# ustcml/RecStudio

Measured on AMD Instinct MI355X. Metric: M scored (user,pos,neg) triplets/sec at d=128, higher is better.
Workload: dtype f32; 1 GPU; BPR two-tower d=128, synthetic 10000001 items / 1000001 users / 1e8-interaction Zipf popularity, positives uniform over the items it holds, popular sampler neg=64, InnerProduct + BPR loss, B=65536 queries/step (BASELINE.json configs[1]); global_batch=65536, num_neg=64, dim=128, n_items=10000001, parallelism=single

## Files before the change

include/recstudio_amd.h:

```cpp
#ifndef RECSTUDIO_AMD_H
#define RECSTUDIO_AMD_H

#include <stdint.h>

#ifdef __cplusplus
extern "C" {
#endif

#define RSA_ABI_VERSION 12

typedef void* rsa_stream_t;

enum rsa_status {
  RSA_OK = 0,
  RSA_ERR_ARG = -1,
  RSA_ERR_HIP = -2,
  RSA_ERR_UNSUPPORTED = -3
};

enum rsa_score_mode { RSA_SCORE_IP = 0, RSA_SCORE_COS = 1, RSA_SCORE_EUC = 2  };
enum rsa_sampler_kind { RSA_SAMPLER_GIVEN = 0, RSA_SAMPLER_UNIFORM = 1, RSA_SAMPLER_POPULAR = 2 };
enum rsa_loss_kind { RSA_LOSS_BPR = 0, RSA_LOSS_SSM = 1, RSA_LOSS_BCE = 2,
                      RSA_LOSS_WBPR = 3, RSA_LOSS_WBCE = 4, RSA_LOSS_HINGE = 5, RSA_LOSS_NCE = 6,
                     RSA_LOSS_CCL = 7 };
// ... 197 lines not shown
  int32_t _pad;
  const rsa_popular_args* pop;
  uint64_t seed, offset;
  uint32_t grid_threads;
  uint32_t _pad2;
  uint64_t elem_base;
  const float* step_scale;
  int64_t* neg_ids;
  uint8_t* solo;
  void* item_workspace;
  int64_t item_workspace_bytes;
  void* user_workspace;
  int64_t user_workspace_bytes;
  float* pos_score;
  float* neg_score;
  float* row_loss;
  float* dpos;
  float* dneg;
  float* query_grad;
  const float* ones;
  float* loss_out;
  void* reduce_scratch;
  int64_t uniform_high;
} rsa_bpr_sgd_args;
int rsa_bpr_sgd_prepare(const rsa_bpr_sgd_args* args, rsa_stream_t stream);
int rsa_bpr_sgd_apply(const rsa_bpr_sgd_args* args, rsa_stream_t stream);

int rsa_scatter_add_rows(const float* src, const int64_t* ids, int64_t numel, int32_t dim,
                         float* dst, int64_t n_rows, rsa_stream_t stream);

typedef struct rsa_seg_gather_args {
  int64_t size;
  const float* item_table;
  int64_t n_items;
  int32_t dim;
  int32_t max_len;
  const int64_t* flat_item_ids;
  int64_t n_flat;
  const int64_t* seg_start;
  const int64_t* seg_end;
  int64_t n_seg;
  int64_t* out_ids;
  float* out_rows;
  int64_t* out_len;
} rsa_seg_gather_args;
int rsa_seg_gather(const rsa_seg_gather_args* args, rsa_stream_t stream);

int rsa_row_sqnorm(const float* table, int64_t n_rows, int32_t dim, int32_t score_mode, float* out, rsa_stream_t stream);

// ... 212 lines not shown
```

recstudio_amd/_native.py:

```python
import ctypes
import os
import subprocess
from ctypes import (POINTER, Structure, c_char_p, c_double, c_float, c_int, c_int32, c_int64, c_uint32, c_uint64, c_void_p)

HERE = os.path.dirname(os.path.abspath(__file__))
LIB_PATH = os.environ.get('RSA_LIB') or os.path.join(HERE, 'librecstudio_amd.so')
CSRC = os.path.join(HERE, 'csrc')

RSA_OK = 0
SCORE_IP, SCORE_COS, SCORE_EUC = 0, 1, 2
SAMPLER_GIVEN, SAMPLER_UNIFORM, SAMPLER_POPULAR = 0, 1, 2
LOSS_BPR, LOSS_SSM, LOSS_BCE = 0, 1, 2
LOSS_WBPR, LOSS_WBCE, LOSS_HINGE, LOSS_NCE, LOSS_CCL = 3, 4, 5, 6, 7


class NativeError(RuntimeError):
    """A C-ABI call returned a negative status."""


class FusedArgs(Structure):
    _fields_ = [
        ('item_table', c_void_p), ('n_items', c_int64), ('dim', c_int32), ('score_mode', c_int32),
        ('query', c_void_p), ('query_index', c_void_p), ('n_query_rows', c_int64),
        ('pos_ids', c_void_p), ('n_queries', c_int64),
# ... 92 lines not shown
    ]


class RowsUpdateArgs(_Sized):
    _fields_ = [
        ('size', c_int64), ('query', c_void_p), ('query_index', c_void_p), ('n_query_rows', c_int64), ('dim', c_int32),
        ('has_pos', c_int32), ('pos_ids', c_void_p), ('neg_ids', c_void_p), ('n_queries', c_int64), ('num_neg', c_int32),
        ('_pad', c_int32), ('dpos', c_void_p), ('dneg', c_void_p), ('upstream', c_void_p), ('n_items', c_int64),
        ('pad_row', c_int64), ('target', c_void_p), ('exp_avg', c_void_p), ('exp_avg_sq', c_void_p), ('lr', c_double),
        ('beta1', c_double), ('beta2', c_double), ('eps', c_double), ('step', c_int64), ('solo', c_void_p), ('workspace', c_void_p),
        ('workspace_bytes', c_int64),
    ]


class BprSgdArgs(_Sized):
    _fields_ = [
        ('size', c_int64), ('item_table', c_void_p), ('n_items', c_int64), ('user_table', c_void_p), ('n_users', c_int64),
        ('dim', c_int32), ('num_neg', c_int32), ('user_ids', c_void_p), ('pos_ids', c_void_p), ('n_queries', c_int64),
        ('sampler', c_int32), ('_pad', c_int32), ('pop', POINTER(PopularArgs)), ('seed', c_uint64), ('offset', c_uint64),
        ('grid_threads', c_uint32), ('_pad2', c_uint32), ('elem_base', c_uint64), ('step_scale', c_void_p), ('neg_ids', c_void_p),
        ('solo', c_void_p), ('item_workspace', c_void_p), ('item_workspace_bytes', c_int64), ('user_workspace', c_void_p),
        ('user_workspace_bytes', c_int64), ('pos_score', c_void_p), ('neg_score', c_void_p), ('row_loss', c_void_p),
        ('dpos', c_void_p), ('dneg', c_void_p), ('query_grad', c_void_p), ('ones', c_void_p), ('loss_out', c_void_p),
        ('reduce_scratch', c_void_p), ('uniform_high', c_int64),
    ]


class SegGatherArgs(_Sized):
    _fields_ = [
        ('size', c_int64), ('item_table', c_void_p), ('n_items', c_int64), ('dim', c_int32), ('max_len', c_int32),
        ('flat_item_ids', c_void_p), ('n_flat', c_int64), ('seg_start', c_void_p), ('seg_end', c_void_p), ('n_seg', c_int64),
        ('out_ids', c_void_p), ('out_rows', c_void_p), ('out_len', c_void_p),
    ]


class FullscoreArgs(_Sized):
    _fields_ = [
        ('size', c_int64), ('item_table', c_void_p), ('n_items', c_int64), ('dim', c_int32), ('score_mode', c_int32),
        ('query', c_void_p), ('n_query', c_int64), ('scores', c_void_p), ('lse', c_void_p), ('topk_val', c_void_p),
        ('topk_idx', c_void_p), ('k', c_int32), ('_pad', c_int32), ('item_aux', c_void_p), ('query_aux', c_void_p),
        ('workspace', c_void_p), ('workspace_bytes', c_int64),
    ]


STRUCTS = {
    'rsa_fused_args': FusedArgs, 'rsa_backward_args': BackwardArgs, 'rsa_shard_route_args': ShardRouteArgs,
    'rsa_shard_home_args': ShardHomeArgs, 'rsa_shard_backward_args': ShardBackwardArgs,
# ... 13 lines not shown
    'rsa_sample_popular': (c_int, [POINTER(PopularArgs), c_void_p]),
    'rsa_popular_lookup': (c_int, [POINTER(PopularArgs), c_void_p]),
    'rsa_item_logp': (c_int, [c_void_p, c_int64, c_void_p, c_int64, c_void_p, c_void_p]),
    'rsa_embedding_gather': (c_int, [c_void_p, c_int64, c_int32, c_void_p, c_int64, c_void_p, c_void_p]),
    'rsa_fused_sample_gather_score': (c_int, [POINTER(FusedArgs), c_void_p]),
    'rsa_pairwise_loss': (c_int, [POINTER(LossArgs), c_void_p]),
    'rsa_ssm_shared_loss': (c_int, [POINTER(LossArgs), c_void_p]),
    'rsa_mean_rows': (c_int, [c_void_p, c_int64, c_void_p, c_void_p, c_void_p]),
    'rsa_row_lse': (c_int, [c_void_p, c_int64, c_int64, c_void_p, c_void_p, c_float, c_void_p]),
    'rsa_fused_backward': (c_int, [POINTER(BackwardArgs), c_void_p]),
    'rsa_sort_step_elements': (c_int, [POINTER(RowsUpdateArgs), c_void_p]),
    'rsa_rows_update_presorted': (c_int, [POINTER(RowsUpdateArgs), c_void_p]),
    'rsa_scatter_add_rows': (c_int, [c_void_p, c_void_p, c_int64, c_int32, c_void_p, c_int64, c_void_p]),
    'rsa_seg_gather': (c_int, [POINTER(SegGatherArgs), c_void_p]),
    'rsa_fullscore_softmax': (c_int, [c_void_p, c_int64, c_int32, c_void_p, c_int64, c_void_p, c_void_p, c_void_p,
                                      c_void_p]),
    'rsa_fullscore_softmax_dq_workspace_bytes': (c_int64, [c_int64, c_int64, c_int32]),
    'rsa_fullscore_softmax_dq': (c_int, [c_void_p, c_int64, c_int32, c_void_p, c_int64, c_void_p, c_void_p, c_void_p,
                                         c_void_p, c_void_p, c_int64, c_void_p]),
    'rsa_scatter_rows_sorted_workspace_bytes': (c_int64, [c_int64, c_int32, c_int64]),
    'rsa_rows_update_sorted': (c_int, [POINTER(RowsUpdateArgs), c_void_p]),
    'rsa_bpr_sgd_prepare': (c_int, [POINTER(BprSgdArgs), c_void_p]),
    'rsa_bpr_sgd_apply': (c_int, [POINTER(BprSgdArgs), c_void_p]),
    'rsa_probs_t_query': (c_int, [c_void_p, c_int64, c_int64, c_int64, c_void_p, c_int32, c_void_p, c_void_p]),
    'rsa_fullscore_lse_grad_workspace_bytes': (c_int64, [c_int64, c_int64, c_int32]),
    'rsa_fullscore_lse_grad': (c_int, [c_void_p, c_int64, c_int32, c_void_p, c_int64, c_void_p, c_void_p, c_void_p, c_int64, c_void_p]),
    'rsa_fullscore_softmax_dw': (c_int, [c_void_p, c_int64, c_int32, c_void_p, c_int64, c_void_p, c_void_p, c_void_p, c_void_p]),
    'rsa_rng_advance': (c_int, [c_void_p, c_uint64, c_void_p]),
    'rsa_placement_probe': (c_int, [c_void_p, c_int64, c_void_p, c_int64, c_uint32, c_void_p]),
    'rsa_row_topk': (c_int, [c_void_p, c_int64, c_int64, c_int32, c_void_p, c_void_p, c_void_p]),
    'rsa_topk_mask_history': (c_int, [c_void_p, c_void_p, c_int32, c_void_p, c_int32, c_int64, c_int32, c_void_p,
                                      c_void_p, c_void_p]),
    'rsa_shard_count': (c_int, [c_void_p, c_void_p, c_int64, c_int32, c_int64, c_int32, c_void_p, c_void_p]),
    'rsa_shard_route': (c_int, [c_void_p, c_void_p, c_int64, c_int32, c_int64, c_int32, c_int64, c_void_p, c_void_p,
                                c_void_p, c_void_p]),
    'rsa_shard_segment_stride': (c_int64, [c_int64]),
    'rsa_shard_sample_route': (c_int, [POINTER(ShardRouteArgs), c_void_p]),
    'rsa_shard_route_workgroups': (c_int64, [POINTER(ShardRouteArgs)]),
    'rsa_shard_route_query_groups': (c_int32, [c_int32, c_uint32, c_uint64, c_int32, c_int32]),
    'rsa_shard_score_segments': (c_int, [c_void_p, c_int64, c_int32, c_void_p, c_int64, c_void_p, c_int64, c_int64, c_void_p,
                                         c_void_p, c_void_p, c_void_p]),
    'rsa_shard_home': (c_int, [POINTER(ShardHomeArgs), c_void_p]),
    'rsa_shard_scatter_slots': (c_int, [c_void_p, c_void_p, c_void_p, c_int64, c_int32, c_void_p, c_void_p]),
    'rsa_shard_unpack_segments': (c_int, [c_void_p, c_int64, c_int64, c_void_p, c_void_p, c_void_p, c_void_p, c_void_p,
                                          c_void_p]),
    'rsa_shard_backward_workspace_bytes': (c_int64, [c_int64, c_int64, c_int64]),
# ... 66 lines not shown
```

recstudio_amd/csrc/rsa_internal.hpp:

```cpp
#pragma once
#include "rsa_launch.hpp"

namespace rsa {

struct AdamArgs {
  float* exp_avg;
  float* exp_avg_sq;
  float one_minus_beta1, one_minus_beta2, eps, step_size;
};

struct SortedLayout {
  uint64_t *pairs_a, *pairs_b;
  void* temp;
  float *lead_part, *trail_part;
  int32_t* meta;
};

int64_t sorted_workspace_bytes(int64_t max_total);
SortedLayout sorted_layout(void* workspace, int64_t max_total);

int classify_solo(uint64_t* pairs, int64_t total, int64_t pad_row, int64_t drop_key, uint8_t* solo, hipStream_t s, const char* who);

int apply_sorted_segments(const uint64_t* pairs, int64_t total, int64_t slots, const float* query, int32_t dim,
                          const int64_t* keys, const float* d, const float* upstream, int64_t n_rows, int64_t pad_row,
                          float* target, const SortedLayout& L, hipStream_t s);

struct StepDraw;
int64_t step_all_workspace_bytes(int64_t n_queries, int32_t num_neg);
int sort_step_all(const int64_t* pos_ids, int64_t* neg_ids, const int64_t* user_ids, int64_t n_queries, int32_t num_neg,
                  int64_t n_items, int64_t n_users, uint8_t* solo, void* workspace, int64_t workspace_bytes, const StepDraw* draw,
                  hipStream_t s, const char* who);
int apply_step_all(bool users, const float* query, const int64_t* query_index, int32_t dim, int64_t n_queries, int32_t num_neg,
                   const float* dpos, const float* dneg, const float* upstream, int64_t n_items, int64_t n_users, float* target,
                   void* workspace, hipStream_t s);

int sample_popular(const rsa_popular_args& a, rsa_stream_t stream);

}
```

recstudio_amd/csrc/rsa_sorted.hip:

```cpp
#include "rsa_common.hpp"
#include "rsa_radix.hpp"
#include "rsa_internal.hpp"
#include <cstring>

#ifndef RSA_SORTED_UNROLL
#define RSA_SORTED_UNROLL 4
#endif
#ifndef RSA_SORTED_NT
#define RSA_SORTED_NT 2
#endif

namespace rsa {

template <bool NT>
__device__ __forceinline__ float ld_row(const float* p) {
  if constexpr (NT) return __builtin_nontemporal_load(p);
  return *p;
}
template <bool NT>
__device__ __forceinline__ void st_row(float* p, float v) {
  if constexpr (NT) __builtin_nontemporal_store(v, p);
  else *p = v;
}

template <int NDW, bool NT = false>
__device__ __forceinline__ void apply_run(float* __restrict__ target, const AdamArgs& adam, int32_t cur, float scale, int lane,
                                          const float (&acc)[NDW], const float (&trow)[NDW], const float (&mrow_v)[NDW],
                                          const float (&vrow_v)[NDW]) {
  constexpr int D = 64 * NDW;
  float* row = target + (size_t)cur * D;
  if (adam.exp_avg == nullptr) {
#pragma unroll
// ... 94 lines not shown
  uint64_t work = __ballot(in && !solo && key != drop_key && key != pad_row);
  int last_t = -1;
  constexpr int U = RSA_SORTED_UNROLL;
  while (work) {
    int ts[U];
    int nu = 0;
#pragma unroll
    for (int u = 0; u < U; ++u) {
      ts[u] = 63;
      if (work) {
        ts[u] = __ffsll((unsigned long long)work) - 1;
        work &= work - 1;
        nu = u + 1;
      }
    }
    float qv[U][NDW], tv[U][NDW], mv[U][NDW], vv[U][NDW];
#pragma unroll
    for (int u = 0; u < U; ++u) {
      const int32_t qr = u < nu ? __builtin_amdgcn_readlane(qrow, ts[u]) : 0;
      const int32_t kr = u < nu ? __builtin_amdgcn_readlane(key, ts[u]) : 0;
      const float* qp = query + (size_t)qr * D;
      const float* tp = target + (size_t)kr * D;
#pragma unroll
      for (int k = 0; k < NDW; ++k) {
        qv[u][k] = qp[k * 64 + lane];
        tv[u][k] = ld_row<NT>(tp + k * 64 + lane);
      }
      if (adam.exp_avg != nullptr) {
        const float* mp = adam.exp_avg + (size_t)kr * D;
        const float* vp = adam.exp_avg_sq + (size_t)kr * D;
#pragma unroll
        for (int k = 0; k < NDW; ++k) {
          mv[u][k] = ld_row<NT>(mp + k * 64 + lane);
          vv[u][k] = ld_row<NT>(vp + k * 64 + lane);
        }
      } else {
#pragma unroll
        for (int k = 0; k < NDW; ++k) mv[u][k] = vv[u][k] = 0.f;
      }
    }
#pragma unroll
    for (int u = 0; u < U; ++u) {
      if (u >= nu) break;
      const int t = ts[u];
      const int32_t kt = __builtin_amdgcn_readlane(key, t);
      const int32_t before = t == 0 ? prev : __builtin_amdgcn_readlane(key, t - 1);
      const bool head = kt != before;
      if (head) {
        close_segment();
        cur = kt;
// ... 39 lines not shown
                                                            const int32_t* __restrict__ meta) {
  constexpr int D = 64 * NDW;
  const int lane = lane_id();
  const int64_t chunk = (int64_t)blockIdx.x * 4 + (threadIdx.x >> 6);
  if (chunk >= n_chunks) return;
  const int32_t cur = meta[chunk * META_STRIDE + META_TRAIL_KEY];
  if (cur < 0 || cur == pad_row) return;
  const float scale = upstream ? upstream[0] : 1.f;
  float acc[NDW], trow[NDW], mrow_v[NDW], vrow_v[NDW];
#pragma unroll
  for (int k = 0; k < NDW; ++k) {
    acc[k] = trail_part[(size_t)chunk * D + k * 64 + lane];
    trow[k] = target[(size_t)cur * D + k * 64 + lane];
    mrow_v[k] = adam.exp_avg ? adam.exp_avg[(size_t)cur * D + k * 64 + lane] : 0.f;
    vrow_v[k] = adam.exp_avg ? adam.exp_avg_sq[(size_t)cur * D + k * 64 + lane] : 0.f;
  }
  for (int64_t c2 = chunk + 1; c2 < n_chunks; ++c2) {
    if (meta[c2 * META_STRIDE + META_LEAD_KEY] != cur) break;
#pragma unroll
    for (int k = 0; k < NDW; ++k) acc[k] += lead_part[(size_t)c2 * D + k * 64 + lane];
    if (!meta[c2 * META_STRIDE + META_LEAD_FULL]) break;
  }
  apply_run<NDW>(target, adam, cur, scale, lane, acc, trow, mrow_v, vrow_v);
}

constexpr int32_t SOLO_BIT = (int32_t)0x80000000;
template <bool MOSTLY_SOLO>
__global__ __launch_bounds__(256) void classify_solo_kernel(uint64_t* __restrict__ pairs, int64_t total, int32_t pad_row,
                                                            int32_t drop_key, uint8_t* __restrict__ solo) {
  const int64_t stride = (int64_t)gridDim.x * blockDim.x;
  for (int64_t i = (int64_t)blockIdx.x * blockDim.x + threadIdx.x; i < total; i += stride) {
    const uint64_t pr = pairs[i];
    const int32_t k = (int32_t)rdx_key(pr);
    const int32_t before = i > 0 ? (int32_t)rdx_key(pairs[i - 1]) : -1, after = i + 1 < total ? (int32_t)rdx_key(pairs[i + 1]) : -1;
    const uint32_t e = rdx_val(pr);
    if (k != before && k != after && k != pad_row && k != drop_key) {
      if (!MOSTLY_SOLO) solo[e] = 1;
      pairs[i] = pr | (uint64_t)(uint32_t)SOLO_BIT;
    } else if (MOSTLY_SOLO) {
      solo[e] = 0;
    }
  }
}

constexpr int64_t SORTED_SMALL_TOTAL = 1 << 18;
int sorted_chunk_elems(int64_t total) { return total <= SORTED_SMALL_TOTAL ? 16 : 64; }
// ... 88 lines not shown
                "rsa_scatter_rows_sorted_workspace_bytes(n_queries, num_neg + 1, n_items): the user rows are sorted with the item rows)",
                who, (long long)workspace_bytes, (long long)need);
  const SortedLayout L = sorted_layout(workspace, total);
  const unsigned bits = step_all_bits(n_items, n_users);
  const SrcStepIds it{pos_ids, neg_ids, n_items, num_neg, num_neg + 1, 1};
  const StepDraw none{nullptr, 0, 0, PhiloxCall{0, 0, 1, 0}, 0, 0, nullptr, nullptr, nullptr};
  const SrcStepAll<false> rd{it, user_ids, t_items, n_users, (uint32_t)(n_items + 1), none};
  hipError_t err;
  if (draw != nullptr && draw->kind != 0) {
    const SrcStepAll<true> dw{it, user_ids, t_items, n_users, (uint32_t)(n_items + 1), *draw};
    err = radix_sort_pairs2(dw, rd, L.pairs_a, L.pairs_b, total, bits, L.temp, s);
  } else {
    err = radix_sort_pairs(rd, L.pairs_a, L.pairs_b, total, bits, L.temp, s);
  }
  if (err != hipSuccess) {
    rsa::set_error("%s: radix sort failed: %s", who, hipGetErrorString(hipGetLastError()));
    return RSA_ERR_HIP;
  }
  return classify_solo(radix_result(L.pairs_a, L.pairs_b, bits), t_items, 0, n_items, solo, s, who);
}

int apply_step_all(bool users, const float* query, const int64_t* query_index, int32_t dim, int64_t n_queries, int32_t num_neg,
                   const float* dpos, const float* dneg, const float* upstream, int64_t n_items, int64_t n_users, float* target,
                   void* workspace, hipStream_t s) {
  const int64_t t_items = n_queries * (int64_t)(num_neg + 1), total = t_items + n_queries;
  const SortedLayout L = sorted_layout(workspace, total);
  const uint64_t* sorted = radix_result(L.pairs_a, L.pairs_b, step_all_bits(n_items, n_users));
  const AdamArgs none{nullptr, nullptr, 0.f, 0.f, 0.f, 0.f};
  if (!users) {
    const DecStep dec{query_index, dpos, dneg, (int)num_neg, 1};
    return apply_sorted_pairs(sorted, t_items, query, dim, dec, upstream, n_items, 0, target, none, L, s);
  }
  const DecStep dec{nullptr, nullptr, dneg, 1, 0};
  return apply_sorted_pairs(sorted + t_items, n_queries, query, dim, dec, upstream, n_users, 0, target, none, L, s, n_items + 1, t_items);
}

}

using namespace rsa;

extern "C" int64_t rsa_scatter_rows_sorted_workspace_bytes(int64_t n_queries, int32_t num_neg, int64_t n_items) {
  if (n_queries <= 0 || num_neg < 0 || n_items < 1) return 0;
  return sorted_workspace_bytes(n_queries * (int64_t)(num_neg + 1));
}

static uint64_t* step_sorted(const SortedLayout& L, int64_t n_items) {
  return radix_result(L.pairs_a, L.pairs_b, radix_key_bits(n_items + 1));
}

static int sort_step_elements(const rsa_rows_update_args& a, uint8_t* solo, hipStream_t s, const char* who) {
  RSA_CHECK_ARG(a.n_queries >= 0 && a.num_neg >= 1 && a.n_items >= 1 && a.n_items < (1ll << 31), "%s: bad sizes", who);
  if (a.n_queries == 0) return RSA_OK;
  RSA_CHECK_ARG(a.neg_ids != nullptr, "%s: neg_ids is null", who);
  const int has_pos = a.pos_ids != nullptr ? 1 : 0;
  const int64_t total = a.n_queries * (int64_t)(a.num_neg + has_pos);
  RSA_CHECK_ARG(total < (1ll << 31), "%s: more than 2^31 elements", who);
  const int64_t need = rsa_scatter_rows_sorted_workspace_bytes(a.n_queries, a.num_neg, a.n_items);
  RSA_CHECK_ARG(a.workspace && a.workspace_bytes >= need, "%s: workspace too small (%lld < %lld)", who, (long long)a.workspace_bytes,
                (long long)need);
  const SortedLayout L = sorted_layout(a.workspace, a.n_queries * (int64_t)(a.num_neg + 1));
  const SrcStepIds src{a.pos_ids, a.neg_ids, a.n_items, a.num_neg, a.num_neg + has_pos, has_pos};
  if (radix_sort_pairs(src, L.pairs_a, L.pairs_b, total, radix_key_bits(a.n_items + 1), L.temp, s) != hipSuccess) {
    rsa::set_error("%s: radix sort failed: %s", who, hipGetErrorString(hipGetLastError()));
    return RSA_ERR_HIP;
  }
  if (solo != nullptr) return classify_solo(step_sorted(L, a.n_items), total, a.pad_row, a.n_items, solo, s, who);
  return RSA_OK;
}

static AdamArgs adam_of(const rsa_rows_update_args& a) {
  if (a.exp_avg == nullptr) return AdamArgs{nullptr, nullptr, 0.f, 0.f, 0.f, 0.f};
  const double bc1 = 1.0 - pow(a.beta1, (double)a.step), bc2 = 1.0 - pow(a.beta2, (double)a.step);
  return AdamArgs{a.exp_avg, a.exp_avg_sq, (float)(1.0 - a.beta1), (float)(1.0 - a.beta2), (float)a.eps,
                  (float)(a.lr * sqrt(bc2) / bc1)};
}

static int check_adam(const rsa_rows_update_args& a, const char* who) {
  if (a.exp_avg == nullptr && a.exp_avg_sq == nullptr) return RSA_OK;
  RSA_CHECK_ARG(a.exp_avg && a.exp_avg_sq && a.step >= 1 && a.beta1 >= 0.0 && a.beta1 < 1.0 && a.beta2 >= 0.0 && a.beta2 < 1.0,
                "%s: bad optimizer state / hyper-parameters", who);
  return RSA_OK;
}

static int apply_step_elements(const rsa_rows_update_args& a, int has_pos, hipStream_t s) {
  RSA_CHECK_ARG(a.n_queries >= 0 && a.num_neg >= 1 && a.n_items >= 1 && a.n_items < (1ll << 31), "rsa_rows_update_sorted: bad sizes");
  if (a.n_queries == 0) return RSA_OK;
  RSA_CHECK_ARG(a.query && a.dneg && a.target, "rsa_rows_update_sorted: null pointer");
  RSA_CHECK_ARG(!has_pos || a.dpos != nullptr, "rsa_rows_update_sorted: pos_ids without dpos");
  RSA_CHECK_ARG(a.query_index != nullptr || a.n_query_rows >= a.n_queries, "rsa_rows_update_sorted: query has fewer rows than n_queries");
  const int64_t total = a.n_queries * (int64_t)(a.num_neg + has_pos);
  const int64_t need = rsa_scatter_rows_sorted_workspace_bytes(a.n_queries, a.num_neg, a.n_items);
  RSA_CHECK_ARG(a.workspace && a.workspace_bytes >= need, "rsa_rows_update_sorted: workspace too small (%lld < %lld)",
                (long long)a.workspace_bytes, (long long)need);
  const SortedLayout L = sorted_layout(a.workspace, a.n_queries * (int64_t)(a.num_neg + 1));
  const DecStep dec{a.query_index, a.dpos, a.dneg, (int)a.num_neg, has_pos};
  return apply_sorted_pairs(step_sorted(L, a.n_items), total, a.query, a.dim, dec, a.upstream, a.n_items, a.pad_row, a.target,
                            adam_of(a), L, s);
// ... 28 lines not shown
```

recstudio_amd/csrc/rsa_step.hip:

```cpp
#include "rsa_common.hpp"
#include "rsa_radix.hpp"
#include "rsa_internal.hpp"

using namespace rsa;

static int check_step(const rsa_bpr_sgd_args& a, const char* who) {
  RSA_CHECK_ARG(a.n_queries >= 0 && a.n_items >= 2 && a.n_users >= 1 && a.n_items < (1ll << 31) && a.n_users < (1ll << 31),
                "%s: bad sizes", who);
  RSA_CHECK_ARG(a.num_neg == 64, "%s: num_neg = %d: the in-forward update is built for one 64-negative tile per query", who,
                a.num_neg);
  if (a.dim != 64 && a.dim != 128 && a.dim != 256) {
    rsa::set_error("%s: dim=%d: built for dim in {64, 128, 256}", who, a.dim);
    return RSA_ERR_UNSUPPORTED;
  }
  RSA_CHECK_ARG(a.user_ids && a.pos_ids && a.neg_ids && a.solo && a.item_workspace,
                "%s: null pointer (user_ids / pos_ids / neg_ids / solo / item_workspace)", who);
  RSA_CHECK_ARG(a.item_workspace_bytes >= step_all_workspace_bytes(a.n_queries, a.num_neg),
                "%s: item_workspace holds %lld bytes, the step needs rsa_scatter_rows_sorted_workspace_bytes(n_queries, num_neg + 1, "
                "n_items) = %lld (ABI 11: the user rows are sorted with the item rows; user_workspace is no longer used)",
                who, (long long)a.item_workspace_bytes, (long long)step_all_workspace_bytes(a.n_queries, a.num_neg));
  return RSA_OK;
}

extern "C" int rsa_bpr_sgd_prepare(const rsa_bpr_sgd_args* args, rsa_stream_t stream) {
  rsa_bpr_sgd_args a;
  if (int rc = load_args(a, args, "rsa_bpr_sgd_prepare")) return rc;
  if (int rc = check_step(a, "rsa_bpr_sgd_prepare")) return rc;
  if (a.n_queries == 0) return RSA_OK;
  const int64_t numel = a.n_queries * (int64_t)a.num_neg;
  StepDraw draw{a.neg_ids, 0, 0, PhiloxCall{a.seed, a.offset >> 2, a.grid_threads, a.elem_base}, 0, 0, nullptr, nullptr, nullptr};
  const bool in_sort = a.n_queries * (int64_t)(a.num_neg + 2) > RDX_TILE;
  if (a.sampler == RSA_SAMPLER_UNIFORM) {
    const int64_t high = a.uniform_high > 0 ? a.uniform_high : a.n_items;
    RSA_CHECK_ARG(high >= 2 && high <= a.n_items, "rsa_bpr_sgd_prepare: uniform_high = %lld outside [2, n_items]", (long long)high);
    RSA_CHECK_ARG(a.grid_threads > 0 && (a.offset & 3) == 0, "rsa_bpr_sgd_prepare: bad philox state");
    if (in_sort) {
      draw.kind = 1;
      draw.range = (uint64_t)(high - 1);
      draw.low = 1;
    } else if (int rc = rsa_sample_uniform(a.neg_ids, numel, 1, high, a.seed, a.offset, a.grid_threads, a.elem_base, stream)) {
      return rc;
    }
  } else if (a.sampler == RSA_SAMPLER_POPULAR) {
    rsa_popular_args p;
// ... 14 lines not shown
      p.numel = numel;
      p.seed = a.seed;
      p.offset = a.offset;
      p.grid_threads = a.grid_threads;
      p.elem_base = a.elem_base;
      if (int rc = sample_popular(p, stream)) return rc;
    }
  } else if (a.sampler != RSA_SAMPLER_GIVEN) {
    rsa::set_error("rsa_bpr_sgd_prepare: sampler must be RSA_SAMPLER_GIVEN, RSA_SAMPLER_UNIFORM or RSA_SAMPLER_POPULAR");
    return RSA_ERR_ARG;
  }
  return sort_step_all(a.pos_ids, a.neg_ids, a.user_ids, a.n_queries, a.num_neg, a.n_items, a.n_users, a.solo, a.item_workspace,
                       a.item_workspace_bytes, &draw, (hipStream_t)stream, "rsa_bpr_sgd_prepare");
}

extern "C" int rsa_bpr_sgd_apply(const rsa_bpr_sgd_args* args, rsa_stream_t stream) {
  rsa_bpr_sgd_args a;
  if (int rc = load_args(a, args, "rsa_bpr_sgd_apply")) return rc;
  if (int rc = check_step(a, "rsa_bpr_sgd_apply")) return rc;
  if (a.n_queries == 0) return RSA_OK;
  RSA_CHECK_ARG(a.item_table && a.user_table && a.step_scale && a.pos_score && a.neg_score && a.row_loss && a.dpos && a.dneg &&
                    a.query_grad && a.ones && a.loss_out && a.reduce_scratch,
                "rsa_bpr_sgd_apply: null pointer");
  rsa_fused_args f;
  __builtin_memset(&f, 0, sizeof f);
  f.item_table = a.item_table;
  f.n_items = a.n_items;
  f.dim = a.dim;
  f.score_mode = RSA_SCORE_IP;
  f.query = a.user_table;
  f.query_index = a.user_ids;
  f.n_query_rows = a.n_users;
  f.pos_ids = a.pos_ids;
  f.n_queries = a.n_queries;
  f.num_neg = a.num_neg;
  f.sampler = RSA_SAMPLER_GIVEN;
  f.neg_ids = a.neg_ids;
  f.pos_score = a.pos_score;
  f.neg_score = a.neg_score;
  f.fused_loss = RSA_LOSS_BPR + 1;
  f.row_loss = a.row_loss;
  f.loss_out = a.loss_out;
  f.dpos = a.dpos;
  f.dneg = a.dneg;
  f.query_grad = a.query_grad;
  f.reduce_scratch = a.reduce_scratch;
  f.solo_flags = a.solo;
  f.upd_scale = a.step_scale;
  if (int rc = rsa_fused_sample_gather_score(&f, stream)) return rc;
  if (int rc = apply_step_all(false, a.user_table, a.user_ids, a.dim, a.n_queries, a.num_neg, a.dpos, a.dneg, a.step_scale, a.n_items,
                              a.n_users, a.item_table, a.item_workspace, (hipStream_t)stream))
    return rc;
  return apply_step_all(true, a.query_grad, nullptr, a.dim, a.n_queries, a.num_neg, nullptr, a.ones, a.step_scale, a.n_items, a.n_users,
                        a.user_table, a.item_workspace, (hipStream_t)stream);
}
```

recstudio_amd/fused.py:

```python
import ctypes

import torch

from . import _native as nat
from . import ops, rng
from ._native import ptr
from .sampler import sampler_kind


def _sampler_cfg(sampler, neg_ids, M):
    kind = sampler_kind(sampler) if sampler is not None else nat.SAMPLER_GIVEN
    if kind is None:
        raise TypeError(f'fused path does not cover sampler {type(sampler).__name__}')
    if kind == nat.SAMPLER_GIVEN:
        if neg_ids is None:
            raise ValueError('neg_ids is required when no sampler is given')
        return kind, {'neg_ids': neg_ids.reshape(M, -1)}
    return kind, (sampler.lookup_kwargs() if kind == nat.SAMPLER_POPULAR else {})


_POP_KEYS = ('table', 'pop_prob', 'guide', 'guide_log2', 'table_prob', 'cdf_lut', 'cdf_lines', 'lines_log2')


def _pop_kw(cfg):
# ... 232 lines not shown


def _reserve_draw(a, kind, sampler, M, num_neg, dev):
    pc = rng.reserve(M * num_neg, rng.sampler_unroll(kind, int(sampler.num_items) + 1), dev, None)
    a.seed, a.offset, a.grid_threads, a.elem_base = pc.seed, pc.offset, pc.grid_threads, pc.elem_base


def _popular_block(sampler):
    kw = sampler.lookup_kwargs()
    kw.pop('table_prob', None)
    return ops.popular_args(**kw), kw


def _check_tables(who, iw, uw):
    if not (iw.is_cuda and iw.is_contiguous() and uw.is_contiguous() and uw.device == iw.device and iw.dtype == uw.dtype == torch.float32):
        raise RuntimeError(f'{who}: contiguous fp32 tables on one GPU (there is no CPU fallback)')


def _ids_ok(user_ids, pos_ids, dev):
    return (user_ids.is_cuda and user_ids.dtype == pos_ids.dtype == torch.int64 and user_ids.device == dev
            and pos_ids.numel() == user_ids.numel())


def _bpr_sgd_step_in_forward(item_weight, user_weight, num_neg, lr, user_ids, pos_ids, sampler, kind, kw):
    M = user_ids.numel()
    iw, uw = item_weight.data, user_weight.data
    dev = iw.device
    _check_tables('bpr_sgd_step', iw, uw)
    if not _ids_ok(user_ids, pos_ids, dev):
        raise TypeError('bpr_sgd_step: int64 user / positive ids on the tables\' device, one positive per query')
    user_ids, pos_ids = user_ids.contiguous(), pos_ids.contiguous()
    neg = None
    if kind == nat.SAMPLER_GIVEN:
        neg = kw['neg_ids']
        if not (neg.dtype == torch.int64 and neg.device == dev and neg.shape == (M, num_neg)):
            raise TypeError('bpr_sgd_step: neg_ids must be int64 [n_queries, num_neg] on the tables\' device')
        neg = neg.contiguous()
    with torch.no_grad(), _device_of(dev):
        step = torch.full((1,), -float(lr), dtype=torch.float32, device=dev)
        b = _sgd_step_block(iw, uw, num_neg, M, kind, sampler, step, neg=neg)
        a = b['args']
        if kind == nat.SAMPLER_POPULAR:
            pop, _ = _popular_block(sampler)
            a.pop = ctypes.pointer(pop)
        a.user_ids, a.pos_ids = user_ids.data_ptr(), pos_ids.data_ptr()
        if kind != nat.SAMPLER_GIVEN:
            _reserve_draw(a, kind, sampler, M, num_neg, dev)
        loss = torch.empty((), dtype=torch.float32, device=dev)
        a.loss_out = loss.data_ptr()
        main = torch.cuda.current_stream(dev)
        a.reduce_scratch = ptr(ops._scratch_for(dev, main.cuda_stream))
        lib = nat.lib()
        rc = lib.rsa_bpr_sgd_prepare(b['ref'], main.cuda_stream)
        if rc != 0:
            nat.check(rc, 'rsa_bpr_sgd_prepare')
        rc = lib.rsa_bpr_sgd_apply(b['ref'], main.cuda_stream)
        if rc != 0:
            nat.check(rc, 'rsa_bpr_sgd_apply')
    return loss, b['neg']


class PrefetchedBPRSGD:

    RING = 2

    def __init__(self, item_weight, user_weight, num_neg, lr, sampler):
        self.iw, self.uw = item_weight.data, user_weight.data
        if not (num_neg == 64 and self.iw.shape[1] in (64, 128, 256)):
            raise NotImplementedError('PrefetchedBPRSGD: num_neg == 64 and embed_dim in {64, 128, 256} (the in-forward update)')
        self.kind = sampler_kind(sampler)
        if self.kind not in (nat.SAMPLER_UNIFORM, nat.SAMPLER_POPULAR):
            raise TypeError(f'PrefetchedBPRSGD does not cover sampler {type(sampler).__name__}')
        _check_tables('PrefetchedBPRSGD', self.iw, self.uw)
        self.num_neg, self.sampler, self.dev = int(num_neg), sampler, self.iw.device
        self.side = torch.cuda.Stream(device=self.dev)
        self.step_scale = torch.full((1,), -float(lr), dtype=torch.float32, device=self.dev)
        self._fork = torch.cuda.Event()
        self._slots, self._count = {}, 0
        self._lib = nat.lib()
        self._pop = self._pop_src = None

    def set_lr(self, lr):
        self.step_scale.fill_(-float(lr))

    def _popular_tables(self):
        src = self.sampler._buffers.get('table')
        if self._pop is None or src is not self._pop_src:
            self._pop, self._pop_keep = _popular_block(self.sampler)
            self._pop_src = src
            for slots in self._slots.values():
                for sl in slots:
                    sl['args'].pop = ctypes.pointer(self._pop)
        return self._pop

    def _slot(self, M):
        slots = self._slots.get(M)
        if slots is None:
            slots = []
            for _ in range(self.RING):
# ... 18 lines not shown
        _reserve_draw(a, self.kind, self.sampler, M, self.num_neg, self.dev)
        main = torch.cuda.current_stream(self.dev)
        self._fork.record(main)
        self.side.wait_event(self._fork)
        with _device_of(self.dev):
            rc = self._lib.rsa_bpr_sgd_prepare(b['ref'], self.side.cuda_stream)
        if rc != 0:
            nat.check(rc, 'rsa_bpr_sgd_prepare')
        b['ready'].record(self.side)
        return {'user_ids': user_ids, 'pos_ids': pos_ids, 'neg': b['neg'], 'slot': b, 'seq': self._count}

    def step(self, ticket):
        b = ticket['slot']
        if ticket['seq'] + self.RING <= self._count:
            raise RuntimeError('PrefetchedBPRSGD.step: this ticket\'s buffers were reused (tickets are stepped in order, at most '
                               f'{self.RING - 1} prepared ahead)')
        main = torch.cuda.current_stream(self.dev)
        main.wait_event(b['ready'])
        loss = torch.empty((), dtype=torch.float32, device=self.dev)
        a = b['args']
        a.loss_out = loss.data_ptr()
        with _device_of(self.dev):
            a.reduce_scratch = ptr(ops._scratch_for(self.dev, main.cuda_stream))
            rc = self._lib.rsa_bpr_sgd_apply(b['ref'], main.cuda_stream)
        if rc != 0:
            nat.check(rc, 'rsa_bpr_sgd_apply')
        return loss, ticket['neg']


class _device_of:
    __slots__ = ('dev', 'guard')

    def __init__(self, dev):
        self.dev, self.guard = dev, None

    def __enter__(self):
        if self.dev.index != torch.cuda.current_device():
            self.guard = torch.cuda.device(self.dev)
            self.guard.__enter__()

    def __exit__(self, *exc):
        if self.guard is not None:
            self.guard.__exit__(*exc)


class FusedBPRAdam:

    def __init__(self, item_weight, user_weight, lr=1e-3, betas=(0.9, 0.999), eps=1e-8):
        self.iw, self.uw = item_weight.data, user_weight.data
        if self.iw.shape[1] not in (64, 128, 256):
            raise NotImplementedError('FusedBPRAdam: embed_dim must be 64, 128 or 256')
        self.lr, self.betas, self.eps, self.t = float(lr), betas, float(eps), 0
        self.state = {k: torch.zeros_like(w) for k, w in (('im', self.iw), ('iv', self.iw), ('um', self.uw), ('uv', self.uw))}

    def step(self, num_neg, *, user_ids, pos_ids, sampler=None, neg_ids=None):
        M = user_ids.numel()
        kind, kw = _sampler_cfg(sampler, neg_ids, M)
        self.t += 1
        st = self.state
        with torch.no_grad():
            out = ops.fused_forward(self.iw, self.uw, num_neg, query_index=user_ids, pos_ids=pos_ids, sampler=kind,
                                    want_logp=False, fused_bpr=True, want_query_grad=True, **kw)
            hp = dict(lr=self.lr, betas=self.betas, eps=self.eps, step=self.t)
            ops.adam_rows_sorted(self.iw, st['im'], st['iv'], self.uw, out['neg_ids'], out['dneg'], query_index=user_ids,
                                 pos_ids=pos_ids, dpos=out['dpos'], pad_row=0, **hp)
            ones = torch.ones(M, 1, dtype=torch.float32, device=self.iw.device)
            ops.adam_rows_sorted(self.uw, st['um'], st['uv'], out['query_grad'], user_ids.view(M, 1), ones, pad_row=0, **hp)
        return out['loss'], out['neg_ids']

    def prepare(self, num_neg, *, user_ids, pos_ids, sampler):
        if sampler_kind(sampler) not in (nat.SAMPLER_UNIFORM, nat.SAMPLER_POPULAR):
            raise TypeError(f'FusedBPRAdam.prepare does not cover sampler {type(sampler).__name__}')
        if getattr(self, 'side', None) is None:
            self.side = torch.cuda.Stream(device=self.iw.device)
        main = torch.cuda.current_stream(self.iw.device)
        self.side.wait_stream(main)
        with torch.no_grad(), torch.cuda.stream(self.side):
            neg = sampler(torch.empty(user_ids.numel(), 1, device=self.iw.device), num_neg, None)[0]
            _, ws = ops.sort_step_elements(pos_ids, neg, self.iw.shape[0], pad_row=0, want_solo=False)
            _, ws_user = ops.sort_step_elements(None, user_ids.view(-1, 1), self.uw.shape[0], pad_row=0, want_solo=False)
            ready = torch.cuda.Event()
            ready.record(self.side)
        for t in (neg, ws, ws_user):
            t.record_stream(main)
        return {'user_ids': user_ids, 'pos_ids': pos_ids, 'neg': neg, 'ws': ws, 'ws_user': ws_user, 'ready': ready,
                'num_neg': int(num_neg)}

    def step_prepared(self, ticket):
        torch.cuda.current_stream(self.iw.device).wait_event(ticket['ready'])
        uid, pos, neg, n = ticket['user_ids'], ticket['pos_ids'], ticket['neg'], ticket['num_neg']
        M = uid.numel()
        self.t += 1
        st = self.state
        with torch.no_grad():
            out = ops.fused_forward(self.iw, self.uw, n, query_index=uid, pos_ids=pos, neg_ids=neg, sampler=nat.SAMPLER_GIVEN,
                                    want_logp=False, fused_bpr=True, want_query_grad=True)
            hp = dict(lr=self.lr, betas=self.betas, eps=self.eps, step=self.t)
            ops.adam_rows_presorted(self.iw, st['im'], st['iv'], self.uw, ticket['ws'], M, n, out['dneg'], query_index=uid,
                                    dpos=out['dpos'], pad_row=0, **hp)
            ones = torch.ones(M, 1, dtype=torch.float32, device=self.iw.device)
            ops.adam_rows_presorted(self.uw, st['um'], st['uv'], out['query_grad'], ticket['ws_user'], M, 1, ones, pad_row=0, **hp)
        return out['loss'], out['neg_ids']
```

Measured before the change: 8793 M triplets/s.

## Route fused BPR Adam through prefetched sorted-apply pipeline with solo-row kernel

Adds rsa_bpr_adam_apply, which runs the fused sample/gather/score forward and then applies Adam updates through the sorted step-all path. Rows touched only once in the batch go through a new per-query solo kernel. FusedBPRAdam.step/prepare now use this two-call path, with a prefetch ring, when num_neg is 64. Separately, the sorted apply kernel now skips loading target and moment rows for lanes that do not open a new run, cutting redundant gathers. The cost is a more complex dispatch, and correctness now depends on the solo flags and the sorted run metadata agreeing.

```diff
diff --git a/include/recstudio_amd.h b/include/recstudio_amd.h
--- a/include/recstudio_amd.h
+++ b/include/recstudio_amd.h
@@ -243,9 +243,16 @@
   float* loss_out;
   void* reduce_scratch;
   int64_t uniform_high;
+  float* item_exp_avg;
+  float* item_exp_avg_sq;
+  float* user_exp_avg;
+  float* user_exp_avg_sq;
+  double lr, beta1, beta2, eps;
+  int64_t step;
 } rsa_bpr_sgd_args;
 int rsa_bpr_sgd_prepare(const rsa_bpr_sgd_args* args, rsa_stream_t stream);
 int rsa_bpr_sgd_apply(const rsa_bpr_sgd_args* args, rsa_stream_t stream);
+int rsa_bpr_adam_apply(const rsa_bpr_sgd_args* args, rsa_stream_t stream);
 
 int rsa_scatter_add_rows(const float* src, const int64_t* ids, int64_t numel, int32_t dim,
                          float* dst, int64_t n_rows, rsa_stream_t stream);
diff --git a/recstudio_amd/_native.py b/recstudio_amd/_native.py
--- a/recstudio_amd/_native.py
+++ b/recstudio_amd/_native.py
@@ -138,7 +138,9 @@
         ('solo', c_void_p), ('item_workspace', c_void_p), ('item_workspace_bytes', c_int64), ('user_workspace', c_void_p),
         ('user_workspace_bytes', c_int64), ('pos_score', c_void_p), ('neg_score', c_void_p), ('row_loss', c_void_p),
         ('dpos', c_void_p), ('dneg', c_void_p), ('query_grad', c_void_p), ('ones', c_void_p), ('loss_out', c_void_p),
-        ('reduce_scratch', c_void_p), ('uniform_high', c_int64),
+        ('reduce_scratch', c_void_p), ('uniform_high', c_int64), ('item_exp_avg', c_void_p), ('item_exp_avg_sq', c_void_p),
+        ('user_exp_avg', c_void_p), ('user_exp_avg_sq', c_void_p), ('lr', c_double), ('beta1', c_double), ('beta2', c_double),
+        ('eps', c_double), ('step', c_int64),
     ]
 
 
@@ -198,6 +200,7 @@
     'rsa_rows_update_sorted': (c_int, [POINTER(RowsUpdateArgs), c_void_p]),
     'rsa_bpr_sgd_prepare': (c_int, [POINTER(BprSgdArgs), c_void_p]),
     'rsa_bpr_sgd_apply': (c_int, [POINTER(BprSgdArgs), c_void_p]),
+    'rsa_bpr_adam_apply': (c_int, [POINTER(BprSgdArgs), c_void_p]),
     'rsa_probs_t_query': (c_int, [c_void_p, c_int64, c_int64, c_int64, c_void_p, c_int32, c_void_p, c_void_p]),
     'rsa_fullscore_lse_grad_workspace_bytes': (c_int64, [c_int64, c_int64, c_int32]),
     'rsa_fullscore_lse_grad': (c_int, [c_void_p, c_int64, c_int32, c_void_p, c_int64, c_void_p, c_void_p, c_void_p, c_int64, c_void_p]),
diff --git a/recstudio_amd/csrc/rsa_internal.hpp b/recstudio_amd/csrc/rsa_internal.hpp
--- a/recstudio_amd/csrc/rsa_internal.hpp
+++ b/recstudio_amd/csrc/rsa_internal.hpp
@@ -8,6 +8,11 @@
   float* exp_avg_sq;
   float one_minus_beta1, one_minus_beta2, eps, step_size;
 };
+
+static inline AdamArgs adam_constants(float* exp_avg, float* exp_avg_sq, double lr, double beta1, double beta2, double eps, int64_t step) {
+  const double bc1 = 1.0 - pow(beta1, (double)step), bc2 = 1.0 - pow(beta2, (double)step);
+  return AdamArgs{exp_avg, exp_avg_sq, (float)(1.0 - beta1), (float)(1.0 - beta2), (float)eps, (float)(lr * sqrt(bc2) / bc1)};
+}
 
 struct SortedLayout {
   uint64_t *pairs_a, *pairs_b;
@@ -32,7 +37,10 @@
                   hipStream_t s, const char* who);
 int apply_step_all(bool users, const float* query, const int64_t* query_index, int32_t dim, int64_t n_queries, int32_t num_neg,
                    const float* dpos, const float* dneg, const float* upstream, int64_t n_items, int64_t n_users, float* target,
-                   void* workspace, hipStream_t s);
+                   void* workspace, hipStream_t s, const AdamArgs& adam = AdamArgs{nullptr, nullptr, 0.f, 0.f, 0.f, 0.f});
+int apply_solo_rows(const float* query, const int64_t* query_index, int64_t n_query_rows, int32_t dim, int64_t n_queries,
+                    const int64_t* pos_ids, const int64_t* neg_ids, const uint8_t* solo, const float* dpos, const float* dneg,
+                    int64_t n_items, float* target, const AdamArgs& adam, hipStream_t s);
 
 int sample_popular(const rsa_popular_args& a, rsa_stream_t stream);
 
diff --git a/recstudio_amd/csrc/rsa_sorted.hip b/recstudio_amd/csrc/rsa_sorted.hip
--- a/recstudio_amd/csrc/rsa_sorted.hip
+++ b/recstudio_amd/csrc/rsa_sorted.hip
@@ -8,6 +8,9 @@
 #endif
 #ifndef RSA_SORTED_NT
 #define RSA_SORTED_NT 2
+#endif
+#ifndef RSA_SORTED_HEAD_ROWS
+#define RSA_SORTED_HEAD_ROWS 1
 #endif
 
 namespace rsa {
@@ -148,10 +151,17 @@
       const float* qp = query + (size_t)qr * D;
       const float* tp = target + (size_t)kr * D;
 #pragma unroll
-      for (int k = 0; k < NDW; ++k) {
-        qv[u][k] = qp[k * 64 + lane];
-        tv[u][k] = ld_row<NT>(tp + k * 64 + lane);
+      for (int k = 0; k < NDW; ++k) qv[u][k] = qp[k * 64 + lane];
+#if RSA_SORTED_HEAD_ROWS
+      const bool opens = u < nu && kr != (ts[u] == 0 ? prev : __builtin_amdgcn_readlane(key, ts[u] > 0 ? ts[u] - 1 : 0));
+      if (!opens) {
+#pragma unroll
+        for (int k = 0; k < NDW; ++k) tv[u][k] = mv[u][k] = vv[u][k] = 0.f;
+        continue;
       }
+#endif
+#pragma unroll
+      for (int k = 0; k < NDW; ++k) tv[u][k] = ld_row<NT>(tp + k * 64 + lane);
       if (adam.exp_avg != nullptr) {
         const float* mp = adam.exp_avg + (size_t)kr * D;
         const float* vp = adam.exp_avg_sq + (size_t)kr * D;
@@ -237,6 +247,75 @@
     if (!meta[c2 * META_STRIDE + META_LEAD_FULL]) break;
   }
   apply_run<NDW>(target, adam, cur, scale, lane, acc, trow, mrow_v, vrow_v);
+}
+
+template <int NDW, bool NT>
+__global__ __launch_bounds__(256) void solo_apply_kernel(const float* __restrict__ query, const int64_t* __restrict__ query_index,
+                                                         int64_t n_queries, const int64_t* __restrict__ pos_ids,
+                                                         const int64_t* __restrict__ neg_ids, const uint8_t* __restrict__ solo,
+                                                         const float* __restrict__ dpos, const float* __restrict__ dneg,
+                                                         int64_t n_query_rows, int64_t n_items, float* __restrict__ target, AdamArgs adam) {
+  constexpr int D = 64 * NDW;
+  constexpr int U = NDW > 2 ? 4 : 8;
+  const int lane = lane_id();
+  const int64_t m = (int64_t)blockIdx.x * 4 + (threadIdx.x >> 6);
+  if (m >= n_queries) return;
+  const int64_t nid = neg_ids[m * 64 + lane], pid = pos_ids[m];
+  const float ncf = dneg[m * 64 + lane];
+  uint64_t work = __ballot(solo[m * 65 + 1 + lane] != 0 && nid > 0 && nid < n_items);
+  bool pos_work = solo[m * 65] != 0 && pid > 0 && pid < n_items;
+  if (work == 0 && !pos_work) return;
+  const int64_t qr = query_index[m];
+  if (qr < 0 || qr >= n_query_rows) return;
+  const float pcf = dpos[m];
+  const int32_t nrow = (int32_t)nid;
+  float q[NDW];
+#pragma unroll
+  for (int k = 0; k < NDW; ++k) q[k] = query[(size_t)qr * D + k * 64 + lane];
+  while (work || pos_work) {
+    int32_t rows[U];
+    float cfs[U];
+    int nu = 0;
+#pragma unroll
+    for (int u = 0; u < U; ++u) {
+      rows[u] = 0;
+      cfs[u] = 0.f;
+      if (pos_work) {
+        rows[u] = (int32_t)pid;
+        cfs[u] = pcf;
+        pos_work = false;
+        nu = u + 1;
+      } else if (work) {
+        const int t = __ffsll((unsigned long long)work) - 1;
+        work &= work - 1;
+        rows[u] = __builtin_amdgcn_readlane(nrow, t);
+        cfs[u] = __int_as_float(__builtin_amdgcn_readlane(__float_as_int(ncf), t));
+        nu = u + 1;
+      }
+    }
+    float tv[U][NDW], mv[U][NDW], vv[U][NDW];
+#pragma unroll
+    for (int u = 0; u < U; ++u) {
+      if (u >= nu) break;
+      const float* tp = target + (size_t)rows[u] * D;
+      const float* mp = adam.exp_avg + (size_t)rows[u] * D;
+      const float* vp = adam.exp_avg_sq + (size_t)rows[u] * D;
+#pragma unroll
+      for (int k = 0; k < NDW; ++k) {
+        tv[u][k] = ld_row<NT>(tp + k * 64 + lane);
+        mv[u][k] = ld_row<NT>(mp + k * 64 + lane);
+        vv[u][k] = ld_row<NT>(vp + k * 64 + lane);
+      }
+    }
+#pragma unroll
+    for (int u = 0; u < U; ++u) {
+      if (u >= nu) break;
+      float acc[NDW];
+#pragma unroll
+      for (int k = 0; k < NDW; ++k) acc[k] = __fmaf_rn(cfs[u], q[k], 0.f);
+      apply_run<NDW, NT>(target, adam, rows[u], 1.f, lane, acc, tv[u], mv[u], vv[u]);
+    }
+  }
 }
 
 constexpr int32_t SOLO_BIT = (int32_t)0x80000000;
@@ -371,17 +450,35 @@
 
 int apply_step_all(bool users, const float* query, const int64_t* query_index, int32_t dim, int64_t n_queries, int32_t num_neg,
                    const float* dpos, const float* dneg, const float* upstream, int64_t n_items, int64_t n_users, float* target,
-                   void* workspace, hipStream_t s) {
+                   void* workspace, hipStream_t s, const AdamArgs& adam) {
   const int64_t t_items = n_queries * (int64_t)(num_neg + 1), total = t_items + n_queries;
   const SortedLayout L = sorted_layout(workspace, total);
   const uint64_t* sorted = radix_result(L.pairs_a, L.pairs_b, step_all_bits(n_items, n_users));
-  const AdamArgs none{nullptr, nullptr, 0.f, 0.f, 0.f, 0.f};
   if (!users) {
     const DecStep dec{query_index, dpos, dneg, (int)num_neg, 1};
-    return apply_sorted_pairs(sorted, t_items, query, dim, dec, upstream, n_items, 0, target, none, L, s);
+    return apply_sorted_pairs(sorted, t_items, query, dim, dec, upstream, n_items, 0, target, adam, L, s);
   }
   const DecStep dec{nullptr, nullptr, dneg, 1, 0};
-  return apply_sorted_pairs(sorted + t_items, n_queries, query, dim, dec, upstream, n_users, 0, target, none, L, s, n_items + 1, t_items);
+  return apply_sorted_pairs(sorted + t_items, n_queries, query, dim, dec, upstream, n_users, 0, target, adam, L, s, n_items + 1, t_items);
+}
+
+int apply_solo_rows(const float* query, const int64_t* query_index, int64_t n_query_rows, int32_t dim, int64_t n_queries,
+                    const int64_t* pos_ids, const int64_t* neg_ids, const uint8_t* solo, const float* dpos, const float* dneg,
+                    int64_t n_items, float* target, const AdamArgs& adam, hipStream_t s) {
+  const bool nt = RSA_SORTED_NT == 1 || (RSA_SORTED_NT == 2 && streams_past_cache(n_items, dim));
+  const dim3 grid((unsigned)((n_queries + 3) / 4)), block(256);
+  const bool built = dispatch_dim<64, 128, 256>(dim, [&](auto D) {
+    dispatch_bool(nt, [&](auto NT) {
+      hipLaunchKernelGGL((solo_apply_kernel<D() / 64, NT()>), grid, block, 0, s, query, query_index, n_queries, pos_ids, neg_ids, solo,
+                         dpos, dneg, n_query_rows, n_items, target, adam);
+    });
+  });
+  if (!built) {
+    rsa::set_error("rsa_bpr_adam_apply: dim=%d: built for dim in {64, 128, 256}", dim);
+    return RSA_ERR_UNSUPPORTED;
+  }
+  RSA_CHECK_LAUNCH("rsa_bpr_adam_apply(solo rows)");
+  return RSA_OK;
 }
 
 }
@@ -419,9 +516,7 @@
 
 static AdamArgs adam_of(const rsa_rows_update_args& a) {
   if (a.exp_avg == nullptr) return AdamArgs{nullptr, nullptr, 0.f, 0.f, 0.f, 0.f};
-  const double bc1 = 1.0 - pow(a.beta1, (double)a.step), bc2 = 1.0 - pow(a.beta2, (double)a.step);
-  return AdamArgs{a.exp_avg, a.exp_avg_sq, (float)(1.0 - a.beta1), (float)(1.0 - a.beta2), (float)a.eps,
-                  (float)(a.lr * sqrt(bc2) / bc1)};
+  return adam_constants(a.exp_avg, a.exp_avg_sq, a.lr, a.beta1, a.beta2, a.eps, a.step);
 }
 
 static int check_adam(const rsa_rows_update_args& a, const char* who) {
diff --git a/recstudio_amd/csrc/rsa_step.hip b/recstudio_amd/csrc/rsa_step.hip
--- a/recstudio_amd/csrc/rsa_step.hip
+++ b/recstudio_amd/csrc/rsa_step.hip
@@ -20,6 +20,33 @@
                 "n_items) = %lld (ABI 11: the user rows are sorted with the item rows; user_workspace is no longer used)",
                 who, (long long)a.item_workspace_bytes, (long long)step_all_workspace_bytes(a.n_queries, a.num_neg));
   return RSA_OK;
+}
+
+static rsa_fused_args step_forward(const rsa_bpr_sgd_args& a) {
+  rsa_fused_args f;
+  __builtin_memset(&f, 0, sizeof f);
+  f.item_table = a.item_table;
+  f.n_items = a.n_items;
+  f.dim = a.dim;
+  f.score_mode = RSA_SCORE_IP;
+  f.query = a.user_table;
+  f.query_index = a.user_ids;
+  f.n_query_rows = a.n_users;
+  f.pos_ids = a.pos_ids;
+  f.n_queries = a.n_queries;
+  f.num_neg = a.num_neg;
+  f.sampler = RSA_SAMPLER_GIVEN;
+  f.neg_ids = a.neg_ids;
+  f.pos_score = a.pos_score;
+  f.neg_score = a.neg_score;
+  f.fused_loss = RSA_LOSS_BPR + 1;
+  f.row_loss = a.row_loss;
+  f.loss_out = a.loss_out;
+  f.dpos = a.dpos;
+  f.dneg = a.dneg;
+  f.query_grad = a.query_grad;
+  f.reduce_scratch = a.reduce_scratch;
+  return f;
 }
 
 extern "C" int rsa_bpr_sgd_prepare(const rsa_bpr_sgd_args* args, rsa_stream_t stream) {
@@ -80,29 +107,7 @@
   RSA_CHECK_ARG(a.item_table && a.user_table && a.step_scale && a.pos_score && a.neg_score && a.row_loss && a.dpos && a.dneg &&
                     a.query_grad && a.ones && a.loss_out && a.reduce_scratch,
                 "rsa_bpr_sgd_apply: null pointer");
-  rsa_fused_args f;
-  __builtin_memset(&f, 0, sizeof f);
-  f.item_table = a.item_table;
-  f.n_items = a.n_items;
-  f.dim = a.dim;
-  f.score_mode = RSA_SCORE_IP;
-  f.query = a.user_table;
-  f.query_index = a.user_ids;
-  f.n_query_rows = a.n_users;
-  f.pos_ids = a.pos_ids;
-  f.n_queries = a.n_queries;
-  f.num_neg = a.num_neg;
-  f.sampler = RSA_SAMPLER_GIVEN;
-  f.neg_ids = a.neg_ids;
-  f.pos_score = a.pos_score;
-  f.neg_score = a.neg_score;
-  f.fused_loss = RSA_LOSS_BPR + 1;
-  f.row_loss = a.row_loss;
-  f.loss_out = a.loss_out;
-  f.dpos = a.dpos;
-  f.dneg = a.dneg;
-  f.query_grad = a.query_grad;
-  f.reduce_scratch = a.reduce_scratch;
+  rsa_fused_args f = step_forward(a);
   f.solo_flags = a.solo;
   f.upd_scale = a.step_scale;
   if (int rc = rsa_fused_sample_gather_score(&f, stream)) return rc;
@@ -112,3 +117,29 @@
   return apply_step_all(true, a.query_grad, nullptr, a.dim, a.n_queries, a.num_neg, nullptr, a.ones, a.step_scale, a.n_items, a.n_users,
                         a.user_table, a.item_workspace, (hipStream_t)stream);
 }
+
+extern "C" int rsa_bpr_adam_apply(const rsa_bpr_sgd_args* args, rsa_stream_t stream) {
+  rsa_bpr_sgd_args a;
+  if (int rc = load_args(a, args, "rsa_bpr_adam_apply")) return rc;
+  if (int rc = check_step(a, "rsa_bpr_adam_apply")) return rc;
+  RSA_CHECK_ARG(a.item_exp_avg && a.item_exp_avg_sq && a.user_exp_avg && a.user_exp_avg_sq && a.step >= 1 && a.beta1 >= 0.0 &&
+                    a.beta1 < 1.0 && a.beta2 >= 0.0 && a.beta2 < 1.0,
+                "rsa_bpr_adam_apply: bad optimizer state / hyper-parameters");
+  if (a.n_queries == 0) return RSA_OK;
+  RSA_CHECK_ARG(a.item_table && a.user_table && a.pos_score && a.neg_score && a.row_loss && a.dpos && a.dneg && a.query_grad &&
+                    a.ones && a.loss_out && a.reduce_scratch,
+                "rsa_bpr_adam_apply: null pointer");
+  hipStream_t s = (hipStream_t)stream;
+  rsa_fused_args f = step_forward(a);
+  if (int rc = rsa_fused_sample_gather_score(&f, stream)) return rc;
+  const AdamArgs items = adam_constants(a.item_exp_avg, a.item_exp_avg_sq, a.lr, a.beta1, a.beta2, a.eps, a.step);
+  const AdamArgs users = adam_constants(a.user_exp_avg, a.user_exp_avg_sq, a.lr, a.beta1, a.beta2, a.eps, a.step);
+  if (int rc = apply_solo_rows(a.user_table, a.user_ids, a.n_users, a.dim, a.n_queries, a.pos_ids, a.neg_ids, a.solo, a.dpos, a.dneg,
+                               a.n_items, a.item_table, items, s))
+    return rc;
+  if (int rc = apply_step_all(false, a.user_table, a.user_ids, a.dim, a.n_queries, a.num_neg, a.dpos, a.dneg, nullptr, a.n_items,
+                              a.n_users, a.item_table, a.item_workspace, s, items))
+    return rc;
+  return apply_step_all(true, a.query_grad, nullptr, a.dim, a.n_queries, a.num_neg, nullptr, a.ones, nullptr, a.n_items, a.n_users,
+                        a.user_table, a.item_workspace, s, users);
+}
diff --git a/recstudio_amd/fused.py b/recstudio_amd/fused.py
--- a/recstudio_amd/fused.py
+++ b/recstudio_amd/fused.py
@@ -278,24 +278,27 @@
             and pos_ids.numel() == user_ids.numel())
 
 
-def _bpr_sgd_step_in_forward(item_weight, user_weight, num_neg, lr, user_ids, pos_ids, sampler, kind, kw):
+def _bpr_sgd_step_in_forward(item_weight, user_weight, num_neg, lr, user_ids, pos_ids, sampler, kind, kw, who='bpr_sgd_step',
+                             apply='rsa_bpr_sgd_apply', fill=None):
     M = user_ids.numel()
     iw, uw = item_weight.data, user_weight.data
     dev = iw.device
-    _check_tables('bpr_sgd_step', iw, uw)
+    _check_tables(who, iw, uw)
     if not _ids_ok(user_ids, pos_ids, dev):
-        raise TypeError('bpr_sgd_step: int64 user / positive ids on the tables\' device, one positive per query')
+        raise TypeError(f'{who}: int64 user / positive ids on the tables\' device, one positive per query')
     user_ids, pos_ids = user_ids.contiguous(), pos_ids.contiguous()
     neg = None
     if kind == nat.SAMPLER_GIVEN:
         neg = kw['neg_ids']
         if not (neg.dtype == torch.int64 and neg.device == dev and neg.shape == (M, num_neg)):
-            raise TypeError('bpr_sgd_step: neg_ids must be int64 [n_queries, num_neg] on the tables\' device')
+            raise TypeError(f'{who}: neg_ids must be int64 [n_queries, num_neg] on the tables\' device')
         neg = neg.contiguous()
     with torch.no_grad(), _device_of(dev):
-        step = torch.full((1,), -float(lr), dtype=torch.float32, device=dev)
+        step = None if lr is None else torch.full((1,), -float(lr), dtype=torch.float32, device=dev)
         b = _sgd_step_block(iw, uw, num_neg, M, kind, sampler, step, neg=neg)
         a = b['args']
+        if fill is not None:
+            fill(a)
         if kind == nat.SAMPLER_POPULAR:
             pop, _ = _popular_block(sampler)
             a.pop = ctypes.pointer(pop)
@@ -310,15 +313,16 @@
         rc = lib.rsa_bpr_sgd_prepare(b['ref'], main.cuda_stream)
         if rc != 0:
             nat.check(rc, 'rsa_bpr_sgd_prepare')
-        rc = lib.rsa_bpr_sgd_apply(b['ref'], main.cuda_stream)
+        rc = getattr(lib, apply)(b['ref'], main.cuda_stream)
         if rc != 0:
-            nat.check(rc, 'rsa_bpr_sgd_apply')
+            nat.check(rc, apply)
     return loss, b['neg']
 
 
 class PrefetchedBPRSGD:
 
     RING = 2
+    APPLY = 'rsa_bpr_sgd_apply'
 
     def __init__(self, item_weight, user_weight, num_neg, lr, sampler):
         self.iw, self.uw = item_weight.data, user_weight.data
@@ -331,6 +335,7 @@
         self.num_neg, self.sampler, self.dev = int(num_neg), sampler, self.iw.device
         self.side = torch.cuda.Stream(device=self.dev)
         self.step_scale = torch.full((1,), -float(lr), dtype=torch.float32, device=self.dev)
+        self._apply = getattr(nat.lib(), self.APPLY)
         self._fork = torch.cuda.Event()
         self._slots, self._count = {}, 0
         self._lib = nat.lib()
@@ -395,10 +400,14 @@
         a.loss_out = loss.data_ptr()
         with _device_of(self.dev):
             a.reduce_scratch = ptr(ops._scratch_for(self.dev, main.cuda_stream))
-            rc = self._lib.rsa_bpr_sgd_apply(b['ref'], main.cuda_stream)
+            self._fill(a)
+            rc = self._apply(b['ref'], main.cuda_stream)
         if rc != 0:
-            nat.check(rc, 'rsa_bpr_sgd_apply')
+            nat.check(rc, self.APPLY)
         return loss, ticket['neg']
+
+    def _fill(self, a):
+        """what a step sets in the block beyond the batch (nothing for SGD: the rate lives in the device scalar)"""
 
 
 class _device_of:
@@ -417,19 +426,40 @@
             self.guard.__exit__(*exc)
 
 
+class _AdamAhead(PrefetchedBPRSGD):
+    APPLY = 'rsa_bpr_adam_apply'
+
+    def __init__(self, owner, num_neg, sampler):
+        super().__init__(owner.iw, owner.uw, num_neg, 0.0, sampler)
+        self._fill = owner._adam_fields
+
+
 class FusedBPRAdam:
 
-    def __init__(self, item_weight, user_weight, lr=1e-3, betas=(0.9, 0.999), eps=1e-8):
+    def __init__(self, item_weight, user_weight, lr=1e-3, betas=(0.9, 0.999), eps=1e-8, solo_rows=True):
         self.iw, self.uw = item_weight.data, user_weight.data
         if self.iw.shape[1] not in (64, 128, 256):
             raise NotImplementedError('FusedBPRAdam: embed_dim must be 64, 128 or 256')
         self.lr, self.betas, self.eps, self.t = float(lr), betas, float(eps), 0
+        self.solo_rows = bool(solo_rows)
         self.state = {k: torch.zeros_like(w) for k, w in (('im', self.iw), ('iv', self.iw), ('um', self.uw), ('uv', self.uw))}
+        self._ahead = {}
+
+    def _adam_fields(self, a):
+        st = self.state
+        a.item_exp_avg, a.item_exp_avg_sq, a.user_exp_avg, a.user_exp_avg_sq = ptr(st['im']), ptr(st['iv']), ptr(st['um']), ptr(st['uv'])
+        a.lr, a.beta1, a.beta2, a.eps, a.step = self.lr, float(self.betas[0]), float(self.betas[1]), self.eps, self.t
+
+    def _two_calls(self, num_neg, user_ids, pos_ids):
+        return self.solo_rows and int(num_neg) == 64 and _ids_ok(user_ids, pos_ids, self.iw.device)
 
     def step(self, num_neg, *, user_ids, pos_ids, sampler=None, neg_ids=None):
         M = user_ids.numel()
         kind, kw = _sampler_cfg(sampler, neg_ids, M)
         self.t += 1
+        if self._two_calls(num_neg, user_ids, pos_ids):
+            return _bpr_sgd_step_in_forward(self.iw, self.uw, int(num_neg), None, user_ids, pos_ids, sampler, kind, kw,
+                                            who='FusedBPRAdam.step', apply='rsa_bpr_adam_apply', fill=self._adam_fields)
         st = self.state
         with torch.no_grad():
             out = ops.fused_forward(self.iw, self.uw, num_neg, query_index=user_ids, pos_ids=pos_ids, sampler=kind,
@@ -444,6 +474,13 @@
     def prepare(self, num_neg, *, user_ids, pos_ids, sampler):
         if sampler_kind(sampler) not in (nat.SAMPLER_UNIFORM, nat.SAMPLER_POPULAR):
             raise TypeError(f'FusedBPRAdam.prepare does not cover sampler {type(sampler).__name__}')
+        if self._two_calls(num_neg, user_ids, pos_ids) and user_ids.is_contiguous() and pos_ids.is_contiguous():
+            ahead = self._ahead.get(id(sampler))
+            if ahead is None or ahead.sampler is not sampler:
+                ahead = self._ahead[id(sampler)] = _AdamAhead(self, int(num_neg), sampler)
+            ticket = ahead.prepare(user_ids, pos_ids)
+            ticket['ahead'] = ahead
+            return ticket
         if getattr(self, 'side', None) is None:
             self.side = torch.cuda.Stream(device=self.iw.device)
         main = torch.cuda.current_stream(self.iw.device)
@@ -460,6 +497,9 @@
                 'num_neg': int(num_neg)}
 
     def step_prepared(self, ticket):
+        if 'ahead' in ticket:
+            self.t += 1
+            return ticket['ahead'].step(ticket)
         torch.cuda.current_stream(self.iw.device).wait_event(ticket['ready'])
         uid, pos, neg, n = ticket['user_ids'], ticket['pos_ids'], ticket['neg'], ticket['num_neg']
         M = uid.numel()
```

Measured after the change: 8792 M triplets/s. No clear change (-0.0%).
